# GradientSpaces/LivingScenes

Hardware: AMD Instinct MI355X
Metric: object-instances/sec (encode+match+register), N=1024 pts (higher is better)
Workload: dtype f32 (GEMM products as two-piece f16 splits on the f16 matrix cores, fp32 accumulate: as accurate against fp64 as an fp32 FMA chain)

## Files before the change

livingscenes_amd/csrc/knn_mfma.hip:

```cpp
#include "knn_common.h"
#include "ls_launch.h"

namespace ls {


template <int CC>
struct QuadRow {
    float4 v[6];
    __device__ __forceinline__ void load(const float* __restrict__ row, int lane, int round = 0) {
        const int off = round * 32 + (lane & 3) * 8;
#pragma unroll
        for (int x = 0; x < 3; ++x)
#pragma unroll
            for (int h = 0; h < 2; ++h) v[x * 2 + h] = *reinterpret_cast<const float4*>(row + x * CC + off + 4 * h);
    }
};
template <int CC, bool FMA, bool LAST>
__device__ __forceinline__ float quad_round(float d, const QuadRow<CC>& q, const QuadRow<CC>& c) {
#pragma clang fp contract(off)
    float t[24];
#pragma unroll
    for (int h = 0; h < 2; ++h)
#pragma unroll
        for (int x = 0; x < 3; ++x) {
            const float4 a = q.v[x * 2 + h], b = c.v[x * 2 + h];
            const float d0 = a.x - b.x, d1 = a.y - b.y, d2 = a.z - b.z, d3 = a.w - b.w;
            t[(h * 4 + 0) * 3 + x] = FMA ? d0 : d0 * d0;
            t[(h * 4 + 1) * 3 + x] = FMA ? d1 : d1 * d1;
            t[(h * 4 + 2) * 3 + x] = FMA ? d2 : d2 * d2;
            t[(h * 4 + 3) * 3 + x] = FMA ? d3 : d3 * d3;
        }
#pragma unroll
    for (int s = 0; s < 4; ++s) {
#pragma unroll
        for (int j = 0; j < 24; ++j) d = FMA ? __builtin_fmaf(t[j], t[j], d) : d + t[j];
        if (s < 3)
            d = __int_as_float(__builtin_amdgcn_update_dpp(0, __float_as_int(d), 0x90, 0xF, 0xF, false));
        else if (!LAST)
            d = __int_as_float(__builtin_amdgcn_update_dpp(0, __float_as_int(d), 0x93, 0xF, 0xF, false));
    }
    return d;
}
template <int CC, bool FMA>
__device__ __forceinline__ float quad_pair_distance(const QuadRow<CC>& q0, const float* __restrict__ qrow, const float* __restrict__ crow,
                                                    int lane) {
    QuadRow<CC> c;
    c.load(crow, lane, 0);
    if constexpr (CC == 32) {
        return quad_round<CC, FMA, true>(0.0f, q0, c);
    } else {
        float d = quad_round<CC, FMA, false>(0.0f, q0, c);
#pragma unroll
        for (int r = 1; r < CC / 32; ++r) {
            QuadRow<CC> q;
            q.load(qrow, lane, r);
            c.load(crow, lane, r);
            d = (r == CC / 32 - 1) ? quad_round<CC, FMA, true>(d, q, c) : quad_round<CC, FMA, false>(d, q, c);
        }
        return d;
    }
}

constexpr int KNN_CENTRE_ROWS = 16;
template <int KK, int WPT>
__global__ __launch_bounds__(64 * WPT) void knn_prep_f16_tile_kernel(const float* __restrict__ f, const float* __restrict__ fc, int Nc, int N, int Npad,
                                                                    unsigned short* __restrict__ out, float* __restrict__ norms, float* __restrict__ iscale,
                                                                    int32_t* __restrict__ zero_buf, long long zero_n) {
    constexpr int D = KK * 16, KPW = KK / WPT, DW = KPW * 16;
    static_assert(KK % WPT == 0 && DW <= 64, "a wave's dims fit one lane each for the centre");
    __shared__ __attribute__((aligned(16))) float lmu[WPT][64];
    __shared__ float lamax[WPT][32], lsum[WPT][32];
    for (long long i = (long long)blockIdx.x * (64 * WPT) + threadIdx.x; i < zero_n; i += (long long)gridDim.x * (64 * WPT)) zero_buf[i] = 0;
    const int lane = threadIdx.x & 63, w = __builtin_amdgcn_readfirstlane(threadIdx.x >> 6), j = lane & 31, h = lane >> 5;
    const int tpi = Npad >> 5, b = blockIdx.x / tpi, tile = blockIdx.x % tpi, r = tile * 32 + j;
    const bool live = r < N;
    const float* rp = f + ((size_t)b * N + (live ? r : 0)) * D + w * DW + h * 8;
    float4 x[KPW][2];
#pragma unroll
    for (int kk = 0; kk < KPW; ++kk) { x[kk][0] = *reinterpret_cast<const float4*>(rp + kk * 16); x[kk][1] = *reinterpret_cast<const float4*>(rp + kk * 16 + 4); }
    {
        const int nc = min(Nc, KNN_CENTRE_ROWS);
        const float* cp = fc + (size_t)b * Nc * D + w * DW + lane;
        if (lane < DW) {
            float s0 = 0.f, s1 = 0.f, s2 = 0.f, s3 = 0.f;
            for (int rr = 0; rr + 3 < nc; rr += 4) {
                s0 += cp[(size_t)rr * D]; s1 += cp[(size_t)(rr + 1) * D]; s2 += cp[(size_t)(rr + 2) * D]; s3 += cp[(size_t)(rr + 3) * D];
            }
            for (int rr = nc & ~3; rr < nc; ++rr) s0 += cp[(size_t)rr * D];
            lmu[w][lane] = ((s0 + s1) + (s2 + s3)) / (float)nc;
        }
        __builtin_amdgcn_s_waitcnt(0xc07f);
        __builtin_amdgcn_wave_barrier();
    }
    float c[KPW][8];
    float amax = 0.f;
#pragma unroll
    for (int kk = 0; kk < KPW; ++kk) {
        const float4 m0 = *reinterpret_cast<const float4*>(&lmu[w][kk * 16 + h * 8]), m1 = *reinterpret_cast<const float4*>(&lmu[w][kk * 16 + h * 8 + 4]);
        const float4 x0 = x[kk][0], x1 = x[kk][1];
        const float t[8] = {x0.x - m0.x, x0.y - m0.y, x0.z - m0.z, x0.w - m0.w, x1.x - m1.x, x1.y - m1.y, x1.z - m1.z, x1.w - m1.w};
#pragma unroll
        for (int i = 0; i < 8; ++i) { c[kk][i] = live ? t[i] : 0.f; amax = fmaxf(amax, fabsf(t[i])); }
    }
    amax = fmaxf(amax, __shfl_xor(amax, 32, 64));
    if (h == 0) lamax[w][j] = amax;
    __syncthreads();
#pragma unroll
    for (int u = 0; u < WPT; ++u) amax = fmaxf(amax, lamax[u][j]);
    float sc;
    const unsigned be = pow2_scale_be(amax, sc);
    sc = live ? sc : 0.f;
    unsigned short* op = out + ((((size_t)b * tpi + tile) * KK + w * KPW) * 64 + lane) * 8;
    float s = 0.f;
#pragma unroll
    for (int kk = 0; kk < KPW; ++kk) {
        unsigned pk[4];
#pragma unroll
        for (int i = 0; i < 4; ++i) {
            const float c0 = c[kk][2 * i], c1 = c[kk][2 * i + 1];
            s += c0 * c0 + c1 * c1;
            const f16x2_t hv = __builtin_convertvector(f32x2_t{c0 * sc, c1 * sc}, f16x2_t);
            pk[i] = __builtin_bit_cast(unsigned, hv);
        }
        uint4 wv;
        wv.x = pk[0]; wv.y = pk[1]; wv.z = pk[2]; wv.w = pk[3];
        *reinterpret_cast<uint4*>(op + (size_t)kk * 512) = wv;
    }
    s += __shfl_xor(s, 32, 64);
    if (h == 0) lsum[w][j] = s;
    __syncthreads();
    if (w == 0 && h == 0 && live) {
        float t = lsum[0][j];
#pragma unroll
        for (int u = 1; u < WPT; ++u) t += lsum[u][j];
        norms[(size_t)b * N + r] = t;
        iscale[(size_t)b * N + r] = pow2_inv(be);
    }
}
#ifndef LS_KF_PK
#define LS_KF_PK 1
#endif
constexpr int KF_QT = 32;
constexpr int KF_WAVES = 8;
constexpr int KF_LCAP = 64;
constexpr int KF_MAXNS = KF_WAVES * 4 * 32;

template <int CC>
struct KfLds {
    float qrows[KF_QT][3 * CC];
    float qnx[KF_QT], qny[KF_QT];
    unsigned hm[KF_QT][64];
    float T[KF_QT];
    int cnt[KF_QT];
    int base[KF_QT + 1];
    unsigned short list[KF_QT][KF_LCAP];
    unsigned plist[KF_QT * KF_LCAP];
    u64 keys[KF_QT][KF_LCAP];
};

template <int CC, bool FMA>
__device__ __noinline__ u64 kf_brute_row(const float* __restrict__ qrow, const float* __restrict__ sbase, int Ns, int lane) {
    constexpr int RF = 3 * CC;
    const int quad = lane >> 2;
    const bool qlast = (lane & 3) == 3;
    QuadRow<CC> qv;
    qv.load(qrow, lane);
    u64 best = ~0ull;
    for (int base = 0; base < Ns; base += 48) {
        u64 ks[3];
#pragma unroll
        for (int u = 0; u < 3; ++u) {
            const int c = base + u * 16 + quad;
            const bool v = c < Ns;
            ks[u] = make_key(quad_pair_distance<CC, FMA>(qv, qrow, sbase + (size_t)(v ? c : 0) * RF, lane), c, v & qlast);
        }
        const int src = ((lane & 15) << 2) + 3;
        const u64 n0 = bperm64(src, ks[0]), n1 = bperm64(src, ks[1]), n2 = bperm64(src, ks[2]);
        u64 k = lane < 16 ? best : (lane < 32 ? n0 : (lane < 48 ? n1 : n2));
        LS_SORT64(cx64, k, lane)
        best = k;
    }
    return best;
}

template <int CC, bool FMA, int TPW>
__global__ __launch_bounds__(64 * KF_WAVES, FMA ? 3 : 4) void knn_fused_kernel(const float* __restrict__ dstf, const float* __restrict__ srcf, const int32_t* __restrict__ dst_rows,
                                                                  const unsigned short* __restrict__ dq, const unsigned short* __restrict__ sq,
                                                                  const float* __restrict__ nrm_dst, const float* __restrict__ nrm_src,
                                                                  const float* __restrict__ isc_dst, const float* __restrict__ isc_src, int Nd, int dst_n,
                                                                  int dst_npad, int Ns, int ns_pad, int K, int qtiles, float eps,
                                                                  int32_t* __restrict__ idx_out, float* __restrict__ dist_out, int32_t* __restrict__ surv_cnt) {
    constexpr int D = 3 * CC, KK = D / 16, RF = 3 * CC;
    __shared__ __attribute__((aligned(16))) KfLds<CC> L;
    const int tid = threadIdx.x, lane = tid & 63;
    const int wave = __builtin_amdgcn_readfirstlane(tid >> 6);
    const int l31 = lane & 31, lh = lane >> 5;
    const int logical = xcd_remap(blockIdx.x, gridDim.x);
    const int b = logical / qtiles, q0 = (logical - b * qtiles) * KF_QT;
    const unsigned short* dqb = dq + (size_t)b * dst_npad * D;
    const unsigned short* sqb = sq + (size_t)b * ns_pad * D;
    const float* sbase = srcf + (size_t)b * Ns * RF;
    const float* dbase = dstf + (size_t)b * dst_n * RF;
    const int ntiles = ns_pad >> 5;

    for (int i = tid; i < KF_QT * (RF / 4); i += 64 * KF_WAVES) {
        const int qr = i / (RF / 4), c4 = i - qr * (RF / 4);
        const int q = min(q0 + qr, Nd - 1);
        const int r = dst_rows ? dst_rows[(size_t)b * Nd + q] : q;
        *reinterpret_cast<float4*>(&L.qrows[qr][c4 * 4]) = *reinterpret_cast<const float4*>(dbase + (size_t)r * RF + c4 * 4);
    }
    if (tid < KF_QT) {
        const int q = q0 + tid;
        const int r = q < Nd ? (dst_rows ? dst_rows[(size_t)b * Nd + q] : q) : 0;
        const float nq = nrm_dst[(size_t)b * dst_n + r], iq = isc_dst[(size_t)b * dst_n + r];
        L.qnx[tid] = q < Nd ? nq : 0.f;
        L.qny[tid] = q < Nd ? -2.0f * iq : 0.f;
        L.cnt[tid] = 0;
    }
    for (int i = tid; i < KF_QT * 64; i += 64 * KF_WAVES) (&L.hm[0][0])[i] = 0x7F800000u;

    f16x8_t a[KK];
    {
        const int qi = q0 + l31;
        const int r = qi < Nd ? (dst_rows ? dst_rows[(size_t)b * Nd + qi] : qi) : 0;
        const unsigned short* ap = dqb + ((size_t)(r >> 5) * KK * 64 + lh * 32 + (r & 31)) * 8;
#pragma unroll
        for (int kk = 0; kk < KK; ++kk) a[kk] = __builtin_bit_cast(f16x8_t, *reinterpret_cast<const uint4*>(ap + (size_t)kk * 512));
    }
    f32x16_t S[TPW];
    float cns[TPW], cic[TPW];
    {
        f16x8_t bf[2][KK];
        auto load_b = [&](int t, f16x8_t (&dstb)[KK]) {
            const int tg = min(wave + KF_WAVES * t, ntiles - 1);
            const unsigned short* bp = sqb + ((size_t)tg * KK * 64 + lane) * 8;
#pragma unroll
            for (int kk = 0; kk < KK; ++kk) dstb[kk] = __builtin_bit_cast(f16x8_t, *reinterpret_cast<const uint4*>(bp + (size_t)kk * 512));
        };
        load_b(0, bf[0]);
#pragma unroll
        for (int t = 0; t < TPW; ++t) {
            if (t + 1 < TPW) load_b(t + 1, bf[(t + 1) & 1]);
            const int cg = min((wave + KF_WAVES * t) * 32 + l31, Ns - 1);
            cns[t] = nrm_src[(size_t)b * Ns + cg];
            cic[t] = isc_src[(size_t)b * Ns + cg];
#pragma unroll
            for (int r = 0; r < 16; ++r) S[t][r] = 0.0f;
#pragma unroll
            for (int kk = 0; kk < KK; ++kk) S[t] = __builtin_amdgcn_mfma_f32_32x32x16_f16(a[kk], bf[t & 1][kk], S[t], 0, 0, 0);
        }
    }
    __syncthreads();
    bool colv[TPW];
#pragma unroll
    for (int t = 0; t < TPW; ++t) colv[t] = (wave + KF_WAVES * t) < ntiles && (wave + KF_WAVES * t) * 32 + l31 < Ns;
#if LS_KF_PK
    {
        const int slot = (wave & 1) * 32 + l31;
        f32x2_t cn2[TPW], ci2[TPW];
#pragma unroll
        for (int t = 0; t < TPW; ++t) { const float cn = colv[t] ? cns[t] : INFINITY; cn2[t] = f32x2_t{cn, cn}; ci2[t] = f32x2_t{cic[t], cic[t]}; }
        const f32x2_t eps2 = {eps, eps};
#pragma unroll
        for (int r = 0; r < 16; r += 2) {
            const int qr = (r & 3) + 8 * (r >> 2) + 4 * lh;
            const f32x2_t qx = *reinterpret_cast<const f32x2_t*>(&L.qnx[qr]), qy = *reinterpret_cast<const f32x2_t*>(&L.qny[qr]);
            float hm0 = INFINITY, hm1 = INFINITY;
#pragma unroll
            for (int t = 0; t < TPW; ++t) {
                const f32x2_t nn = qx + cn2[t], w = qy * ci2[t];
                const f32x2_t sv = {S[t][r], S[t][r + 1]};
                const f32x2_t dh = __builtin_elementwise_fma(sv, w, nn), e = eps2 * nn;
                const f32x2_t hi = dh + e;
                f32x2_t lo = dh - e;
                hm0 = fminf(hm0, hi.x); hm1 = fminf(hm1, hi.y);
                asm volatile("" : "+v"(lo));
                S[t][r] = lo.x; S[t][r + 1] = lo.y;
            }
            const float h0 = fmaxf(hm0, 0.0f), h1 = fmaxf(hm1, 0.0f);
            if (h0 < INFINITY) atomicMin(&L.hm[qr][slot], __float_as_uint(h0));
            if (h1 < INFINITY) atomicMin(&L.hm[qr + 1][slot], __float_as_uint(h1));
            if ((r & 3) == 2) __builtin_amdgcn_sched_barrier(0);
        }
    }
#else
    {
        const int slot = (wave & 1) * 32 + l31;
#pragma unroll
        for (int r = 0; r < 16; ++r) {
            const int qr = (r & 3) + 8 * (r >> 2) + 4 * lh;
            const float2 qn = make_float2(L.qnx[qr], L.qny[qr]);
            float hmin = INFINITY;
#pragma unroll
            for (int t = 0; t < TPW; ++t) {
                const float nn = qn.x + cns[t], w = qn.y * cic[t];
                const float dh = __builtin_fmaf(S[t][r], w, nn), e = eps * nn;
                hmin = colv[t] ? fminf(hmin, dh + e) : hmin;
                float lo = dh - e;
                asm volatile("" : "+v"(lo));
                S[t][r] = lo;
            }
            const float h = fmaxf(hmin, 0.0f);
            if (h < INFINITY) atomicMin(&L.hm[qr][slot], __float_as_uint(h));
            if ((r & 3) == 3) __builtin_amdgcn_sched_barrier(0);
        }
    }
#endif
    __syncthreads();
#pragma unroll
    for (int u = 0; u < KF_QT / KF_WAVES; ++u) {
        const int qr = wave * (KF_QT / KF_WAVES) + u;
        const unsigned tb = kth_smallest_upper_bound(L.hm[qr][lane], K < 64 ? K : 64);
        if (lane == 0) L.T[qr] = __uint_as_float(tb);
    }
    __syncthreads();
    {
        unsigned mask[TPW];
#pragma unroll
        for (int t = 0; t < TPW; ++t) mask[t] = 0;
#pragma unroll
        for (int r = 0; r < 16; ++r) {
            const float Tr = L.T[(r & 3) + 8 * (r >> 2) + 4 * lh];
#pragma unroll
            for (int t = 0; t < TPW; ++t) mask[t] |= (S[t][r] > Tr) ? 0u : (1u << r);
        }
#pragma unroll
        for (int t = 0; t < TPW; ++t) {
            const int cg = (wave + KF_WAVES * t) * 32 + l31;
            unsigned m = colv[t] ? mask[t] : 0u;
            while (m) {
                const int r = __builtin_ctz(m);
                m &= m - 1;
                const int qr = (r & 3) + 8 * (r >> 2) + 4 * lh;
                if (q0 + qr < Nd) {
                    const int pos = atomicAdd(&L.cnt[qr], 1);
                    if (pos < KF_LCAP) L.list[qr][pos] = (unsigned short)cg;
                }
            }
        }
    }
    __syncthreads();
    if (wave == 0) {
        const int c = (lane < KF_QT && L.cnt[lane] <= KF_LCAP) ? L.cnt[lane] : 0;
        int incl = c;
#pragma unroll
        for (int o = 1; o < KF_QT; o <<= 1) {
            const int v = __shfl_up(incl, o, 64);
            incl += lane >= o ? v : 0;
        }
        if (lane < KF_QT) L.base[lane] = incl - c;
        if (lane == KF_QT - 1) L.base[KF_QT] = incl;
        if (lane < KF_QT && q0 + lane < Nd && surv_cnt) surv_cnt[(size_t)b * Nd + q0 + lane] = -(L.cnt[lane] > KF_LCAP ? Ns : L.cnt[lane]) - 1;
    }
    __syncthreads();
    for (int i = tid; i < KF_QT * KF_LCAP; i += 64 * KF_WAVES) {
        const int qr = i / KF_LCAP, j = i - qr * KF_LCAP;
        const int c = L.cnt[qr];
        if (c <= KF_LCAP && j < c) L.plist[L.base[qr] + j] = (unsigned)L.list[qr][j] | ((unsigned)qr << 16) | ((unsigned)j << 21);
    }
    __syncthreads();
    {
        const int P = L.base[KF_QT];
        const int Q = wave * 16 + (lane >> 2);
        const bool qlast = (lane & 3) == 3;
        struct Pair { unsigned ent; bool v; QuadRow<CC> c; };
        auto fetch = [&](int p0, Pair& pr) {
            const int p = p0 + Q;
            pr.v = p < P;
            pr.ent = L.plist[pr.v ? p : 0];
            pr.c.load(sbase + (size_t)(pr.ent & 0xFFFFu) * RF, lane, 0);
        };
        auto finish = [&](const Pair& pr) {
            const int cand = pr.ent & 0xFFFFu, qr = (pr.ent >> 16) & 31, slot = pr.ent >> 21;
            const float* qrow = &L.qrows[qr][0];
            QuadRow<CC> qv;
            qv.load(qrow, lane);
            float d;
            if constexpr (CC == 32) {
                d = quad_round<CC, FMA, true>(0.0f, qv, pr.c);
            } else {
                const float* crow = sbase + (size_t)cand * RF;
                d = quad_round<CC, FMA, false>(0.0f, qv, pr.c);
#pragma unroll
                for (int r = 1; r < CC / 32; ++r) {
                    QuadRow<CC> q, c;
                    q.load(qrow, lane, r);
                    c.load(crow, lane, r);
                    d = (r == CC / 32 - 1) ? quad_round<CC, FMA, true>(d, q, c) : quad_round<CC, FMA, false>(d, q, c);
                }
            }
            if (pr.v && qlast) L.keys[qr][slot] = make_key(d, cand, true);
        };
        if (P > 0) {
            Pair pa, pb;
            fetch(0, pa);
            for (int p0 = 0; p0 < P; p0 += 2 * 16 * KF_WAVES) {
                fetch(p0 + 16 * KF_WAVES, pb);
                __builtin_amdgcn_sched_barrier(0);
                finish(pa);
                if (p0 + 16 * KF_WAVES < P) {
                    fetch(p0 + 2 * 16 * KF_WAVES, pa);
                    __builtin_amdgcn_sched_barrier(0);
                    finish(pb);
                }
            }
        }
    }
    __syncthreads();
    auto emit = [&](int qr, u64 k, int e) {
        const int q = q0 + qr;
        if (q < Nd && e < K) {
            const size_t o = ((size_t)b * Nd + q) * K + e;
            const unsigned hi = (unsigned)(k >> 32), lw = (unsigned)k;
            idx_out[o] = hi == 0xFFFFFFFFu ? -1 : (int)lw;
            if (dist_out) dist_out[o] = hi == 0xFFFFFFFFu ? INFINITY : __uint_as_float(hi);
        }
    };
#pragma unroll
    for (int u = 0; u < KF_QT / KF_WAVES; u += 2) {
        const int qa = wave * (KF_QT / KF_WAVES) + u, qb = qa + 1;
        const int ca = L.cnt[qa], cb = L.cnt[qb];
        if (ca <= 32 && cb <= 32) {
            const int qr = lh ? qb : qa, c = lh ? cb : ca;
            u64 k = l31 < c ? L.keys[qr][l31] : ~0ull;
            LS_SORT32(cx64, k, lane)
            emit(qr, k, l31);
        } else {
#pragma unroll
            for (int h = 0; h < 2; ++h) {
                const int qr = h ? qb : qa, c = h ? cb : ca;
                u64 k;
                if (c <= KF_LCAP) {
                    k = lane < c ? L.keys[qr][lane] : ~0ull;
                    LS_SORT64(cx64, k, lane)
                } else {
                    k = q0 + qr < Nd ? kf_brute_row<CC, FMA>(&L.qrows[qr][0], sbase, Ns, lane) : ~0ull;
                }
                emit(qr, k, lane);
            }
        }
    }
}

static inline size_t pad32(size_t n) { return (n + 31) & ~(size_t)31; }
static int knn_prep_launch(const float* f, const float* fc, int Nc, int B, int N, int Npad, int D, unsigned short* out, float* norms, float* iscale, hipStream_t st) {
    const int tiles = B * (Npad / 32);
    if (D == 96)
        hipLaunchKernelGGL((knn_prep_f16_tile_kernel<6, 3>), dim3(tiles), dim3(192), 0, st, f, fc, Nc, N, Npad, out, norms, iscale, (int32_t*)nullptr, 0LL);
    else
        hipLaunchKernelGGL((knn_prep_f16_tile_kernel<12, 4>), dim3(tiles), dim3(256), 0, st, f, fc, Nc, N, Npad, out, norms, iscale, (int32_t*)nullptr, 0LL);
    LS_LAUNCH_CHECK();
    return LS_OK;
}
int knn_sweep_max_ns() { return KF_MAXNS; }

struct KfScratch { float *nsrc, *ndst, *isrc, *idst; int32_t* cnt; unsigned short *sq, *dq; size_t bytes; };
static KfScratch kf_layout(void* scratch, int B, int Nd, int dst_n, int Ns, int D, bool self) {
    char* sc = (char*)scratch;
    size_t off = 0;
    auto take = [&](size_t bytes) { char* p = sc + off; off = (off + bytes + 255) & ~(size_t)255; return p; };
    KfScratch k;
    k.cnt = (int32_t*)take((size_t)B * Nd * sizeof(int32_t));
    k.nsrc = (float*)take((size_t)B * Ns * sizeof(float));
    k.ndst = self ? k.nsrc : (float*)take((size_t)B * dst_n * sizeof(float));
    k.isrc = (float*)take((size_t)B * Ns * sizeof(float));
    k.idst = self ? k.isrc : (float*)take((size_t)B * dst_n * sizeof(float));
    k.sq = (unsigned short*)take((size_t)B * pad32(Ns) * D * sizeof(unsigned short));
    k.dq = self ? k.sq : (unsigned short*)take((size_t)B * pad32(dst_n) * D * sizeof(unsigned short));
    k.bytes = off;
    return k;
}
size_t knn_sweep_scratch_bytes(int B, int Nd, int dst_n, int Ns, int C) { return kf_layout(nullptr, B, Nd, dst_n, Ns, 3 * C, false).bytes; }

template <int CC>
static int knn_sweep_launch_t(const float* dst, const float* src, const int32_t* dst_rows, int B, int Nd, int dst_n, int Ns, int K, bool fma,
                              int32_t* idx_out, float* dist_out, void* scratch, hipStream_t st) {
    constexpr int D = 3 * CC;
    const KfScratch k = kf_layout(scratch, B, Nd, dst_n, Ns, D, dst == src);
    const int ns_pad = (int)pad32(Ns), dst_npad = (int)pad32(dst_n);
    int rc = knn_prep_launch(src, src, Ns, B, Ns, ns_pad, D, k.sq, k.nsrc, k.isrc, st);
    if (rc != LS_OK) return rc;
    if (dst != src) {
        rc = knn_prep_launch(dst, src, Ns, B, dst_n, dst_npad, D, k.dq, k.ndst, k.idst, st);
        if (rc != LS_OK) return rc;
    }
    const int qtiles = cdiv(Nd, KF_QT), tpw = cdiv(ns_pad / 32, KF_WAVES);
    const float epsF = 1.02f * 0.0009765625f + 6.0f * (float)(D + 4) * 5.9604645e-8f + 9.5367431640625e-7f + 4.76837158203125e-7f;
#define LS_KF(T) do { if (fma) hipLaunchKernelGGL((knn_fused_kernel<CC, true, T>), dim3(B * qtiles), dim3(64 * KF_WAVES), 0, st, dst, src, dst_rows, k.dq, k.sq, k.ndst, k.nsrc, k.idst, k.isrc, Nd, dst_n, dst_npad, Ns, ns_pad, K, qtiles, epsF, idx_out, dist_out, k.cnt); \
                   else hipLaunchKernelGGL((knn_fused_kernel<CC, false, T>), dim3(B * qtiles), dim3(64 * KF_WAVES), 0, st, dst, src, dst_rows, k.dq, k.sq, k.ndst, k.nsrc, k.idst, k.isrc, Nd, dst_n, dst_npad, Ns, ns_pad, K, qtiles, epsF, idx_out, dist_out, k.cnt); } while (0)
    if (tpw <= 1) LS_KF(1); else if (tpw == 2) LS_KF(2); else LS_KF(4);
#undef LS_KF
    LS_LAUNCH_CHECK();
    return LS_OK;
}

int knn_sweep_launch(const float* dst, const float* src, const int32_t* dst_rows, int B, int Nd, int dst_n, int Ns, int C, int K,
                     bool fma, int32_t* idx_out, float* dist_out, const int32_t* , int , int , void* scratch,
                     hipStream_t st) {
    LS_REQUIRE(C == 32 || C == 64, "knn_sweep: only C == 32 / 64 layers are supported (C=%d)", C);
    LS_REQUIRE((int)pad32(Ns) <= KF_MAXNS && K <= KNN_MAXK, "knn_sweep: Ns=%d K=%d beyond the fused kernel (Ns <= %d, K <= 16)", Ns, K, KF_MAXNS);
    if (C == 32) return knn_sweep_launch_t<32>(dst, src, dst_rows, B, Nd, dst_n, Ns, K, fma, idx_out, dist_out, scratch, st);
    return knn_sweep_launch_t<64>(dst, src, dst_rows, B, Nd, dst_n, Ns, K, fma, idx_out, dist_out, scratch, st);
}

__global__ __launch_bounds__(256) void knn_stats_kernel(const int32_t* __restrict__ surv_cnt, long long nq, unsigned long long* __restrict__ out) {
    unsigned long long s = 0;
    for (long long i = (long long)blockIdx.x * 256 + threadIdx.x; i < nq; i += (long long)gridDim.x * 256) {
        const int c = surv_cnt[i];
        s += (unsigned long long)(c < 0 ? -(c + 1) : 0);
    }
    for (int o = 32; o > 0; o >>= 1) s += __shfl_xor(s, o, 64);
    if ((threadIdx.x & 63) == 0) atomicAdd(&out[0], s);
    if (blockIdx.x == 0 && threadIdx.x == 0) atomicAdd(&out[1], (unsigned long long)nq);
}
int knn_sweep_stats_launch(const void* scratch, int B, int Nd, int dst_n, int Ns, unsigned long long* out, hipStream_t st) {
    const size_t nq = (size_t)B * Nd;
    (void)dst_n; (void)Ns;
    hipLaunchKernelGGL(knn_stats_kernel, dim3((unsigned)std::min<size_t>(cdiv((long long)nq, 256), 256)), dim3(256), 0, st, (const int32_t*)scratch, (long long)nq, out);
    LS_LAUNCH_CHECK();
    return LS_OK;
}

}
```

Measured before the change: 56820.

## Overlap query-row staging with fragment loads and drop prefix-sum barrier round

Moves the staging of query rows and norms into LDS so their global loads are issued alongside the A/B fragment loads, instead of in a separate phase up front. It also replaces the single-wave prefix sum over survivor counts, the base[] array and two block barriers with a per-wave redundant shuffle scan plus readlane, so each wave writes its own packed pair list. An optional timestamp probe, compiled out by default, is added for per-phase timing. The cost is extra redundant scan work in every wave and somewhat more register pressure in the prologue.

After: 56930 (median of 6 runs). About the same (+0.2%).

```diff
diff --git a/livingscenes_amd/csrc/knn_mfma.hip b/livingscenes_amd/csrc/knn_mfma.hip
--- a/livingscenes_amd/csrc/knn_mfma.hip
+++ b/livingscenes_amd/csrc/knn_mfma.hip
@@ -140,6 +140,14 @@
 #ifndef LS_KF_PK
 #define LS_KF_PK 1
 #endif
+#ifdef LS_KF_PROBE
+constexpr int KF_PROBE_PHASES = 9;
+__device__ unsigned long long kf_probe_acc[KF_PROBE_PHASES + 1];
+#define KF_STAMP(i) do { __builtin_amdgcn_sched_barrier(0); asm volatile("s_memtime %0\n\ts_waitcnt lgkmcnt(0)" : "=s"(kf_ts[i]) :: "memory"); \
+                         __builtin_amdgcn_sched_barrier(0); } while (0)
+#else
+#define KF_STAMP(i) do { } while (0)
+#endif
 constexpr int KF_QT = 32;
 constexpr int KF_WAVES = 8;
 constexpr int KF_LCAP = 64;
@@ -152,7 +160,6 @@
     unsigned hm[KF_QT][64];
     float T[KF_QT];
     int cnt[KF_QT];
-    int base[KF_QT + 1];
     unsigned short list[KF_QT][KF_LCAP];
     unsigned plist[KF_QT * KF_LCAP];
     u64 keys[KF_QT][KF_LCAP];
@@ -202,31 +209,27 @@
     const float* sbase = srcf + (size_t)b * Ns * RF;
     const float* dbase = dstf + (size_t)b * dst_n * RF;
     const int ntiles = ns_pad >> 5;
-
-    for (int i = tid; i < KF_QT * (RF / 4); i += 64 * KF_WAVES) {
-        const int qr = i / (RF / 4), c4 = i - qr * (RF / 4);
-        const int q = min(q0 + qr, Nd - 1);
-        const int r = dst_rows ? dst_rows[(size_t)b * Nd + q] : q;
-        *reinterpret_cast<float4*>(&L.qrows[qr][c4 * 4]) = *reinterpret_cast<const float4*>(dbase + (size_t)r * RF + c4 * 4);
-    }
-    if (tid < KF_QT) {
-        const int q = q0 + tid;
-        const int r = q < Nd ? (dst_rows ? dst_rows[(size_t)b * Nd + q] : q) : 0;
-        const float nq = nrm_dst[(size_t)b * dst_n + r], iq = isc_dst[(size_t)b * dst_n + r];
-        L.qnx[tid] = q < Nd ? nq : 0.f;
-        L.qny[tid] = q < Nd ? -2.0f * iq : 0.f;
-        L.cnt[tid] = 0;
-    }
+#ifdef LS_KF_PROBE
+    unsigned long long kf_ts[KF_PROBE_PHASES + 1];
+#endif
+    KF_STAMP(0);
+
+    if (tid < KF_QT) L.cnt[tid] = 0;
     for (int i = tid; i < KF_QT * 64; i += 64 * KF_WAVES) (&L.hm[0][0])[i] = 0x7F800000u;
-
+    KF_STAMP(1);
+
+    constexpr int NROW = (KF_QT * (RF / 4) + 64 * KF_WAVES - 1) / (64 * KF_WAVES);
+    const int qi = q0 + l31;
+    int ra = min(qi, Nd - 1), rp0 = min(q0 + min(tid, KF_QT * (RF / 4) - 1) / (RF / 4), Nd - 1),
+        rp1 = min(q0 + min(tid + 64 * KF_WAVES, KF_QT * (RF / 4) - 1) / (RF / 4), Nd - 1),
+        rp2 = min(q0 + min(tid + 2 * 64 * KF_WAVES, KF_QT * (RF / 4) - 1) / (RF / 4), Nd - 1);
+    if (dst_rows) {
+        const int32_t* dr = dst_rows + (size_t)b * Nd;
+        ra = dr[ra]; rp0 = dr[rp0]; rp1 = dr[rp1];
+        if (NROW > 2) rp2 = dr[rp2];
+    }
+    ra = qi < Nd ? ra : 0;
     f16x8_t a[KK];
-    {
-        const int qi = q0 + l31;
-        const int r = qi < Nd ? (dst_rows ? dst_rows[(size_t)b * Nd + qi] : qi) : 0;
-        const unsigned short* ap = dqb + ((size_t)(r >> 5) * KK * 64 + lh * 32 + (r & 31)) * 8;
-#pragma unroll
-        for (int kk = 0; kk < KK; ++kk) a[kk] = __builtin_bit_cast(f16x8_t, *reinterpret_cast<const uint4*>(ap + (size_t)kk * 512));
-    }
     f32x16_t S[TPW];
     float cns[TPW], cic[TPW];
     {
@@ -237,6 +240,25 @@
 #pragma unroll
             for (int kk = 0; kk < KK; ++kk) dstb[kk] = __builtin_bit_cast(f16x8_t, *reinterpret_cast<const uint4*>(bp + (size_t)kk * 512));
         };
+        const float nq = nrm_dst[(size_t)b * dst_n + ra], iq = isc_dst[(size_t)b * dst_n + ra];
+        constexpr int NPIECE = KF_QT * (RF / 4);
+        const int i0 = tid, i1 = min(tid + 64 * KF_WAVES, NPIECE - 1), i2 = min(tid + 2 * 64 * KF_WAVES, NPIECE - 1);
+        const float4 rv0 = *reinterpret_cast<const float4*>(dbase + (size_t)rp0 * RF + (i0 % (RF / 4)) * 4);
+        const float4 rv1 = *reinterpret_cast<const float4*>(dbase + (size_t)rp1 * RF + (i1 % (RF / 4)) * 4);
+        float4 rv2 = {};
+        if (NROW > 2) rv2 = *reinterpret_cast<const float4*>(dbase + (size_t)rp2 * RF + (i2 % (RF / 4)) * 4);
+        static_assert(NROW == 2 || NROW == 3, "query-row pieces per thread");
+        L.qnx[l31] = qi < Nd ? nq : 0.f;
+        L.qny[l31] = qi < Nd ? -2.0f * iq : 0.f;
+        *reinterpret_cast<float4*>(&L.qrows[0][0] + (size_t)i0 * 4) = rv0;
+        *reinterpret_cast<float4*>(&L.qrows[0][0] + (size_t)i1 * 4) = rv1;
+        if (NROW > 2) *reinterpret_cast<float4*>(&L.qrows[0][0] + (size_t)i2 * 4) = rv2;
+        if (KK > 6) __builtin_amdgcn_sched_barrier(0);
+        {
+            const unsigned short* ap = dqb + ((size_t)(ra >> 5) * KK * 64 + lh * 32 + (ra & 31)) * 8;
+#pragma unroll
+            for (int kk = 0; kk < KK; ++kk) a[kk] = __builtin_bit_cast(f16x8_t, *reinterpret_cast<const uint4*>(ap + (size_t)kk * 512));
+        }
         load_b(0, bf[0]);
 #pragma unroll
         for (int t = 0; t < TPW; ++t) {
@@ -251,6 +273,7 @@
         }
     }
     __syncthreads();
+    KF_STAMP(2);
     bool colv[TPW];
 #pragma unroll
     for (int t = 0; t < TPW; ++t) colv[t] = (wave + KF_WAVES * t) < ntiles && (wave + KF_WAVES * t) * 32 + l31 < Ns;
@@ -307,6 +330,7 @@
     }
 #endif
     __syncthreads();
+    KF_STAMP(3);
 #pragma unroll
     for (int u = 0; u < KF_QT / KF_WAVES; ++u) {
         const int qr = wave * (KF_QT / KF_WAVES) + u;
@@ -314,6 +338,7 @@
         if (lane == 0) L.T[qr] = __uint_as_float(tb);
     }
     __syncthreads();
+    KF_STAMP(4);
     {
         unsigned mask[TPW];
 #pragma unroll
@@ -340,27 +365,29 @@
         }
     }
     __syncthreads();
-    if (wave == 0) {
-        const int c = (lane < KF_QT && L.cnt[lane] <= KF_LCAP) ? L.cnt[lane] : 0;
+    KF_STAMP(5);
+    int P;
+    {
+        const int cl = L.cnt[l31];
+        const int c = cl <= KF_LCAP ? cl : 0;
         int incl = c;
 #pragma unroll
         for (int o = 1; o < KF_QT; o <<= 1) {
-            const int v = __shfl_up(incl, o, 64);
-            incl += lane >= o ? v : 0;
-        }
-        if (lane < KF_QT) L.base[lane] = incl - c;
-        if (lane == KF_QT - 1) L.base[KF_QT] = incl;
-        if (lane < KF_QT && q0 + lane < Nd && surv_cnt) surv_cnt[(size_t)b * Nd + q0 + lane] = -(L.cnt[lane] > KF_LCAP ? Ns : L.cnt[lane]) - 1;
-    }
-    __syncthreads();
-    for (int i = tid; i < KF_QT * KF_LCAP; i += 64 * KF_WAVES) {
-        const int qr = i / KF_LCAP, j = i - qr * KF_LCAP;
-        const int c = L.cnt[qr];
-        if (c <= KF_LCAP && j < c) L.plist[L.base[qr] + j] = (unsigned)L.list[qr][j] | ((unsigned)qr << 16) | ((unsigned)j << 21);
-    }
-    __syncthreads();
-    {
-        const int P = L.base[KF_QT];
+            const int v = __shfl_up(incl, o, 32);
+            incl += l31 >= o ? v : 0;
+        }
+        P = __builtin_amdgcn_readlane(incl, KF_QT - 1);
+        if (wave == 0 && lane < KF_QT && q0 + lane < Nd && surv_cnt) surv_cnt[(size_t)b * Nd + q0 + lane] = -(cl > KF_LCAP ? Ns : cl) - 1;
+#pragma unroll
+        for (int u = 0; u < KF_QT / KF_WAVES; ++u) {
+            const int qr = wave + KF_WAVES * u;
+            const int cq = __builtin_amdgcn_readlane(c, qr), bq = __builtin_amdgcn_readlane(incl, qr) - cq;
+            if (lane < cq) L.plist[bq + lane] = (unsigned)L.list[qr][lane] | ((unsigned)qr << 16) | ((unsigned)lane << 21);
+        }
+    }
+    __syncthreads();
+    KF_STAMP(6);
+    {
         const int Q = wave * 16 + (lane >> 2);
         const bool qlast = (lane & 3) == 3;
         struct Pair { unsigned ent; bool v; QuadRow<CC> c; };
@@ -406,7 +433,9 @@
             }
         }
     }
-    __syncthreads();
+    KF_STAMP(7);
+    __syncthreads();
+    KF_STAMP(8);
     auto emit = [&](int qr, u64 k, int e) {
         const int q = q0 + qr;
         if (q < Nd && e < K) {
@@ -440,6 +469,14 @@
             }
         }
     }
+#ifdef LS_KF_PROBE
+    KF_STAMP(9);
+    if ((blockIdx.x & 127) == 0 && tid == 0) {
+#pragma unroll
+        for (int i = 0; i < KF_PROBE_PHASES; ++i) atomicAdd(&kf_probe_acc[i], kf_ts[i + 1] - kf_ts[i]);
+        atomicAdd(&kf_probe_acc[KF_PROBE_PHASES], 1ull);
+    }
+#endif
 }
 
 static inline size_t pad32(size_t n) { return (n + 31) & ~(size_t)31; }
@@ -522,3 +559,14 @@
 }
 
 }
+
+#ifdef LS_KF_PROBE
+extern "C" int ls_knn_probe_read(unsigned long long* out, int reset) {
+    if (hipMemcpyFromSymbol(out, HIP_SYMBOL(ls::kf_probe_acc), sizeof(ls::kf_probe_acc)) != hipSuccess) return -1;
+    if (reset) {
+        const unsigned long long z[ls::KF_PROBE_PHASES + 1] = {};
+        if (hipMemcpyToSymbol(HIP_SYMBOL(ls::kf_probe_acc), z, sizeof(z)) != hipSuccess) return -1;
+    }
+    return 0;
+}
+#endif
```
